# abstractguy/xagents

Hardware: AMD Instinct MI355X
Metric: env-steps/sec/GPU (PPO 16-env) + update ms; 1/2/4/8 MI355X (higher is better)
Workload: dtype f32; 1 GPU; PPO CartPole-v1, 16 envs/GPU, MLP[64,64], n_steps=128, 4 epochs x 4 minibatches, synthetic obs replay (the metric's 16-env configuration); the replay records ignore the actions, so the rollout runs its policy forwards as one batched launch (the `dynamics` object times the sequential step loop of an action-dependent env); n_envs_per_gpu=16, n_steps=128, batch_per_gpu=2048, minibatch_per_gpu=512, ppo_epochs=4, parallelism=dp1, graph=True, train_steps_per_graph_replay=8, update=persistent, allreduce=none

## Files before the change

### xagents_amd/csrc/ppo_tile.hpp

```cpp
#pragma once
#include <type_traits>

#include "ac_tile.hpp"

namespace xa_pt {

using namespace xa_ac;

template <int OBS, int A, int TS>
struct PtLds {
  static constexpr int AH = A + 1, AHP = (AH + 3) & ~3, LDT = TS + 4;
  alignas(16) float sW2[H * LDW];
  alignas(16) float sH1[TS * LDW];
  alignas(16) float sH1T[H * LDT];
  alignas(16) float sdA2[TS * LDW];
  alignas(16) float sZp[4][TS][AHP];
  alignas(16) float sdz[4][TS][AHP];
  alignas(16) float sW1[OBS * H];
  float sb1[H], sb2[H], sW34[H * AH], sb34[AH];
};

template <int OBS, int A>
XA_DEV int canon_of_exchange(int x) {
  const Offs o = offs(OBS, A);
  if (x < H * H) {
    const int pr = x >> 1, t = pr & 255, kk = 2 * (pr >> 8) + (x & 1);
    const int w = t >> 6, lq = (t >> 4) & 3, li = t & 15;
    return o.w2 + (16 * lq + kk) * H + 16 * w + li;
  }
  const int rr = x - H * H;
  return rr < o.w2 ? rr : rr + H * H;
}

template <int OBS, int A>
XA_DEV int exchange_of_rest(int c) {
  const Offs o = offs(OBS, A);
  return H * H + (c < o.w2 ? c : c - H * H);
}

#ifdef XA_NO_REGH1
constexpr bool kRegH1On = false;
#else
constexpr bool kRegH1On = true;
#endif
template <int OBS, int A>
constexpr bool kRegH1 = kRegH1On && OBS == 4 &&
                        1 + (offs(OBS, A).P - offs(OBS, A).b2 + 191) / 192 <= Dims<OBS, A>::RPT;

template <int OBS, int A, int TS>
struct PSlice {
  static constexpr int RPT = Dims<OBS, A>::RPT, NREST = Dims<OBS, A>::NREST;
  int col, row0;
  int ri[RPT];
  int rx[RPT];
  int rdst[RPT];
  XA_DEV static int rest_of(int tid, int q) {
    const Offs o = offs(OBS, A);
    if constexpr (kRegH1<OBS, A>) {
      const int w = tid >> 6, lane = tid & 63, lq = lane >> 4, li = lane & 15, i = 16 * w + li;
      if (q == 0) return o.w1 + lq * H + i;
      if (lq == 0) return q == 1 ? o.b1 + i : -1;
      const int id2 = (lq - 1) * 64 + 16 * w + li, r2 = id2 + 192 * (q - 1);
      return o.b2 + r2 < o.P ? o.b2 + r2 : -1;
    } else {
      const int r = tid + 256 * q;
      return r < NREST ? (r < o.w2 ? r : r + H * H) : -1;
    }
  }
  XA_DEV void init(int tid) {
    const int w = tid >> 6, lane = tid & 63;
    col = 16 * w + (lane & 15);
    row0 = 16 * (lane >> 4);
#pragma unroll
    for (int q = 0; q < RPT; ++q) {
      const int e = rest_of(tid, q);
      ri[q] = e;
      rx[q] = e >= 0 ? exchange_of_rest<OBS, A>(e) : -1;
      rdst[q] = lds_offset_of<PtLds<OBS, A, TS>, OBS, A>(e);
    }
  }
  XA_DEV int w2_canon(int kk) const { return offs(OBS, A).w2 + (row0 + kk) * H + col; }
  XA_DEV void load(const float* base, float (&w)[16], float (&r)[RPT]) const {
#pragma unroll
    for (int kk = 0; kk < 16; ++kk) w[kk] = base[w2_canon(kk)];
#pragma unroll
    for (int q = 0; q < RPT; ++q) r[q] = base[ri[q] >= 0 ? ri[q] : 0];
  }
  XA_DEV void store(float* base, const float (&w)[16], const float (&r)[RPT]) const {
#pragma unroll
    for (int kk = 0; kk < 16; ++kk) base[w2_canon(kk)] = w[kk];
#pragma unroll
    for (int q = 0; q < RPT; ++q)
      if (ri[q] >= 0) base[ri[q]] = r[q];
  }
  XA_DEV void to_lds(PtLds<OBS, A, TS>& L, const float (&w)[16], const float (&r)[RPT]) const {
#pragma unroll
    for (int kk = 0; kk < 16; ++kk) L.sW2[(row0 + kk) * LDW + col] = w[kk];
#pragma unroll
    for (int q = 0; q < RPT; ++q)
      if (rdst[q] >= 0) reinterpret_cast<float*>(&L)[rdst[q]] = r[q];
  }
};

template <int OBS, int A>
struct PtAcc {
  static constexpr int AH = A + 1;
  f32x4 gW2[4];
  float gW34[AH];
  float gW1[OBS];
  float gb1, gb2;
  float gb34[AH];
  float l_pg, l_v, l_ent, l_cnt;
  XA_DEV void zero() {
#pragma unroll
    for (int it = 0; it < 4; ++it) gW2[it] = f32x4{0.0f, 0.0f, 0.0f, 0.0f};
#pragma unroll
    for (int a = 0; a < AH; ++a) gW34[a] = gb34[a] = 0.0f;
#pragma unroll
    for (int k = 0; k < OBS; ++k) gW1[k] = 0.0f;
    gb1 = gb2 = 0.0f;
    l_pg = l_v = l_ent = l_cnt = 0.0f;
  }
};

XA_DEV xa_f2 ftanh2(xa_f2 x) {
  const float c = kTanhClamp;
  const xa_f2 xc = {fminf(fmaxf(x.x, -c), c), fminf(fmaxf(x.y, -c), c)};
  xa_f2 p, q;
  tanh_pq(xc, xc * xc, p, q);
  const xa_f2 r = {__builtin_amdgcn_rcpf(q.x), __builtin_amdgcn_rcpf(q.y)};
  const xa_f2 rn = xa_fma2(xa_fma2(-q, r, xa_f2{1.0f, 1.0f}), r, r);
  return p * rn;
}

XA_DEV float xa_sum16(float v) {
  v = v + XA_DPP_F(v, 0xB1);
  v = v + XA_DPP_F(v, 0x4E);
  v = v + XA_DPP_F(v, 0x141);
  return v + XA_DPP_F(v, 0x140);
}

template <int OBS, int A, int TS>
XA_DEV void load_w2_rows(const PtLds<OBS, A, TS>& L, float (&w2r)[16]) {
  const int tid = threadIdx.x, w = tid >> 6, li = tid & 15, lq = (tid & 63) >> 4;
#pragma unroll
  for (int v4 = 0; v4 < 4; ++v4) {
    const float4 t = *reinterpret_cast<const float4*>(&L.sW2[(16 * w + li) * LDW + 16 * lq + 4 * v4]);
    w2r[4 * v4] = t.x; w2r[4 * v4 + 1] = t.y; w2r[4 * v4 + 2] = t.z; w2r[4 * v4 + 3] = t.w;
  }
}

XA_DEV float2 xa_swap16(float v) {
  const auto a = __builtin_amdgcn_permlane16_swap(__float_as_uint(v), __float_as_uint(v), false, false);
  return make_float2(__uint_as_float(a[0]), __uint_as_float(a[1]));
}
XA_DEV float2 xa_swap32(float v) {
  const auto a = __builtin_amdgcn_permlane32_swap(__float_as_uint(v), __float_as_uint(v), false, false);
  return make_float2(__uint_as_float(a[0]), __uint_as_float(a[1]));
}

struct PtOwnTid {};
template <class PTid>
XA_DEV void pt_pred_lane(PTid ptid, int& pw, int& pli, int& plq) {
  if constexpr (!std::is_same<PTid, PtOwnTid>::value) {
    pw = ptid >> 6;
    pli = ptid & 15;
    plq = (ptid & 63) >> 4;
  }
}

template <int OBS, int A, int TS, class Stamp, class W2Out, class PTid = PtOwnTid>
XA_DEV void pt_tile(PtLds<OBS, A, TS>& L, PtAcc<OBS, A>& acc, const LossCfg& cfg,
                    const float* rec, const float (&w2c)[16], float (&w2r)[16], float w1v,
                    float b1v, Stamp stamp, bool last, W2Out w2_out, PTid ptid = PTid()) {
  static_assert(TS == 16 || TS == 32, "tile sizes: 16 or 32 samples");
  constexpr int NT = TS / 16, AH = A + 1, R = OBS + 4, LDT = PtLds<OBS, A, TS>::LDT;
  const int tid = threadIdx.x, w = tid >> 6, lane = tid & 63;
  const int li = lane & 15, lq = lane >> 4;
  int pw = w, pli = li, plq = lq;
  pt_pred_lane(ptid, pw, pli, plq);
  const int i = 16 * w + li;
  float h1[NT][4];
  {
    float w1[OBS];
    float b1;
    if constexpr (kRegH1<OBS, A>) {
      const float2 s16 = xa_swap16(w1v), s32 = xa_swap32(w1v);
      float vj[4];
      vj[0] = w1v;
      vj[1] = (plq & 1) ? s16.x : s16.y;
      const float2 s48 = xa_swap32(vj[1]);
      vj[2] = (plq & 2) ? s32.x : s32.y;
      vj[3] = (plq & 2) ? s48.x : s48.y;
      const bool o1 = plq & 1, o2 = plq & 2;
#pragma unroll
      for (int k = 0; k < OBS; ++k) {
        const float e0 = ((k & 1) != 0) != o1 ? vj[1] : vj[0];
        const float e1 = ((k & 1) != 0) != o1 ? vj[3] : vj[2];
        w1[k] = ((k & 2) != 0) != o2 ? e1 : e0;
      }
      b1 = xa_swap32(xa_swap16(b1v).x).x;
    } else {
#pragma unroll
      for (int k = 0; k < OBS; ++k) w1[k] = L.sW1[k * H + i];
      b1 = L.sb1[i];
    }
    stamp(47);
#pragma unroll
    for (int mt = 0; mt < NT; ++mt) {
#pragma unroll
      for (int r = 0; r < 4; r += 2) {
        const int s = 16 * mt + 4 * lq + r;
        xa_f2 z = {0.0f, 0.0f};
#pragma unroll
        for (int k = 0; k < OBS; ++k)
          z = xa_fma2(xa_f2{rec[s * R + k], rec[(s + 1) * R + k]}, xa_f2{w1[k], w1[k]}, z);
        const xa_f2 h = ftanh2(z + xa_f2{b1, b1});
        h1[mt][r] = h.x;
        h1[mt][r + 1] = h.y;
      }
      stamp(48);
#pragma unroll
      for (int r = 0; r < 4; ++r) L.sH1[(16 * mt + 4 * lq + r) * LDW + i] = h1[mt][r];
      *reinterpret_cast<float4*>(&L.sH1T[i * LDT + 16 * mt + 4 * lq]) =
          make_float4(h1[mt][0], h1[mt][1], h1[mt][2], h1[mt][3]);
    }
  }
  stamp(49);
  __syncthreads();
  if constexpr (kRegH1<OBS, A>) load_w2_rows(L, w2r);
  stamp(50);
  float h2[NT][4];
  float w34[AH];
#pragma unroll
  for (int a = 0; a < AH; ++a) w34[a] = L.sW34[i * AH + a];
  {
    const float b2 = L.sb2[i];
#pragma unroll
    for (int mt = 0; mt < NT; ++mt) {
      float av[16];
#pragma unroll
      for (int v4 = 0; v4 < 4; ++v4) {
        const float4 t = *reinterpret_cast<const float4*>(&L.sH1[(16 * mt + li) * LDW + 16 * lq + 4 * v4]);
        av[4 * v4] = t.x; av[4 * v4 + 1] = t.y; av[4 * v4 + 2] = t.z; av[4 * v4 + 3] = t.w;
      }
      f32x4 d0 = {0.0f, 0.0f, 0.0f, 0.0f}, d1 = {0.0f, 0.0f, 0.0f, 0.0f};
#pragma unroll
      for (int kk = 0; kk < 16; kk += 2) {
        d0 = mfma4(av[kk], w2c[kk], d0);
        d1 = mfma4(av[kk + 1], w2c[kk + 1], d1);
      }
#pragma unroll
      for (int r = 0; r < 4; r += 2) {
        const xa_f2 h = ftanh2(xa_f2{d0[r], d0[r + 1]} + xa_f2{d1[r], d1[r + 1]} + xa_f2{b2, b2});
        h2[mt][r] = h.x;
        h2[mt][r + 1] = h.y;
      }
    }
  }
  stamp(51);
#pragma unroll
  for (int mt = 0; mt < NT; ++mt)
#pragma unroll
    for (int r = 0; r < 4; ++r)
#pragma unroll
      for (int a = 0; a < AH; ++a) {
        const float p = xa_sum16(h2[mt][r] * w34[a]);
        if (pli == 0) L.sZp[w][16 * mt + 4 * lq + r][a] = p;
      }
  __syncthreads();
  stamp(52);
  constexpr int AHP = PtLds<OBS, A, TS>::AHP;
  const bool tally = pw == 0 && plq == 0;
#pragma unroll
  for (int mt = 0; mt < NT; ++mt) {
    const int s = 16 * mt + li;
    float z[AHP];
#pragma unroll
    for (int a4 = 0; a4 < AHP; a4 += 4) {
      float4 zp[4];
#pragma unroll
      for (int ww = 0; ww < 4; ++ww) zp[ww] = *reinterpret_cast<const float4*>(&L.sZp[ww][s][a4]);
      z[a4] = (zp[0].x + zp[1].x) + (zp[2].x + zp[3].x);
      z[a4 + 1] = (zp[0].y + zp[1].y) + (zp[2].y + zp[3].y);
      z[a4 + 2] = (zp[0].z + zp[1].z) + (zp[2].z + zp[3].z);
      z[a4 + 3] = (zp[0].w + zp[1].w) + (zp[2].w + zp[3].w);
    }
#pragma unroll
    for (int a = 0; a < AH; ++a) z[a] = z[a] + L.sb34[a];
    const float* rs = rec + s * R;
    const float act_f = rs[OBS];
    float dz[AHP];
#pragma unroll
    for (int a = 0; a < AHP; ++a) dz[a] = 0.0f;
    if (act_f >= 0.0f) {
      const int act = (int)act_f;
      float m = z[0];
#pragma unroll
      for (int a = 1; a < A; ++a) m = fmaxf(m, z[a]);
      float e[A], ssum = 0.0f;
#pragma unroll
      for (int a = 0; a < A; ++a) {
        e[a] = fexp(z[a] - m);
        ssum = ssum + e[a];
      }
      const float ls = flog(ssum), rsum = frcp(ssum);
      float lp[A], pr[A], ent = 0.0f, logp = 0.0f;
#pragma unroll
      for (int a = 0; a < A; ++a) {
        lp[a] = (z[a] - m) - ls;
        pr[a] = e[a] * rsum;
        ent = ent - pr[a] * lp[a];
        if (a == act) logp = lp[a];
      }
      const float v = z[A], R_ = rs[OBS + 1], oldv = rs[OBS + 2];
      const float adv = ((R_ - oldv) - cfg.adv_mean) * cfg.adv_rstd;
      const float ratio = fexp(logp - rs[OBS + 3]);
      const float sc = cfg.loss_scale;
      float pg, dlogp, vl, dv;
      ac_loss_terms(true, adv, ratio, logp, v, oldv, R_, cfg.clip_norm, sc, cfg.value_coef, pg,
                    dlogp, vl, dv);
      const float ec = sc * cfg.entropy_coef;
#pragma unroll
      for (int a = 0; a < A; ++a)
        dz[a] = dlogp * ((a == act ? 1.0f : 0.0f) - pr[a]) + ec * pr[a] * (lp[a] + ent);
      dz[A] = dv;
      if (tally) {
        acc.l_pg += pg;
        acc.l_v += vl;
        acc.l_ent += ent;
        acc.l_cnt += 1.0f;
#pragma unroll
        for (int a = 0; a < AH; ++a) acc.gb34[a] += dz[a];
      }
    }
    if (plq == 0) {
#pragma unroll
      for (int a4 = 0; a4 < AHP; a4 += 4)
        *reinterpret_cast<float4*>(&L.sdz[w][s][a4]) = make_float4(dz[a4], dz[a4 + 1], dz[a4 + 2], dz[a4 + 3]);
    }
  }
  __builtin_amdgcn_fence(__ATOMIC_ACQ_REL, "wavefront");
  float da2[NT][4];
#pragma unroll
  for (int mt = 0; mt < NT; ++mt) {
#pragma unroll
    for (int r = 0; r < 4; ++r) {
      const int s = 16 * mt + 4 * lq + r;
      float dz[AHP];
#pragma unroll
      for (int a4 = 0; a4 < AHP; a4 += 4) {
        const float4 t = *reinterpret_cast<const float4*>(&L.sdz[w][s][a4]);
        dz[a4] = t.x; dz[a4 + 1] = t.y; dz[a4 + 2] = t.z; dz[a4 + 3] = t.w;
      }
      float dh = 0.0f;
#pragma unroll
      for (int a = 0; a < AH; ++a) dh = fmaf(dz[a], w34[a], dh);
      const float hv = h2[mt][r];
#pragma unroll
      for (int a = 0; a < AH; ++a) acc.gW34[a] = fmaf(hv, dz[a], acc.gW34[a]);
      const float d = dh * (1.0f - hv * hv);
      acc.gb2 = acc.gb2 + d;
      da2[mt][r] = d;
      L.sdA2[s * LDW + i] = d;
    }
  }
  stamp(53);
#pragma unroll
  for (int it = 0; it < 4; ++it)
#pragma unroll
    for (int mt = 0; mt < NT; ++mt) {
      const float4 t = *reinterpret_cast<const float4*>(&L.sH1T[(16 * it + li) * LDT + 16 * mt + 4 * lq]);
      acc.gW2[it] = mfma4(t.x, da2[mt][0], acc.gW2[it]);
      acc.gW2[it] = mfma4(t.y, da2[mt][1], acc.gW2[it]);
      acc.gW2[it] = mfma4(t.z, da2[mt][2], acc.gW2[it]);
      acc.gW2[it] = mfma4(t.w, da2[mt][3], acc.gW2[it]);
    }
  if (last) w2_out(acc);
  __syncthreads();
  stamp(54);
#pragma unroll
  for (int mt = 0; mt < NT; ++mt) {
    float av[16];
#pragma unroll
    for (int v4 = 0; v4 < 4; ++v4) {
      const float4 t = *reinterpret_cast<const float4*>(&L.sdA2[(16 * mt + li) * LDW + 16 * lq + 4 * v4]);
      av[4 * v4] = t.x; av[4 * v4 + 1] = t.y; av[4 * v4 + 2] = t.z; av[4 * v4 + 3] = t.w;
    }
    f32x4 d0 = {0.0f, 0.0f, 0.0f, 0.0f}, d1 = {0.0f, 0.0f, 0.0f, 0.0f};
#pragma unroll
    for (int kk = 0; kk < 16; kk += 2) {
      d0 = mfma4(av[kk], w2r[kk], d0);
      d1 = mfma4(av[kk + 1], w2r[kk + 1], d1);
    }
#pragma unroll
    for (int r = 0; r < 4; ++r) {
      const int s = 16 * mt + 4 * lq + r;
      const float hv = h1[mt][r];
      const float d = (d0[r] + d1[r]) * (1.0f - hv * hv);
      acc.gb1 = acc.gb1 + d;
#pragma unroll
      for (int k = 0; k < OBS; ++k) acc.gW1[k] = fmaf(rec[s * R + k], d, acc.gW1[k]);
    }
  }
  stamp(55);
}

template <int OBS, int A, class PutPair>
XA_DEV void pt_write_row_w2(const PtAcc<OBS, A>& acc, PutPair put_pair) {
  const int tid = threadIdx.x, w = tid >> 6, lane = tid & 63;
  const int li = lane & 15, lq = lane >> 4;
#pragma unroll
  for (int it = 0; it < 4; ++it) {
    const int t = 64 * w + 16 * it + li;
    put_pair(256 * (2 * lq) + t, acc.gW2[it][0], acc.gW2[it][1]);
    put_pair(256 * (2 * lq + 1) + t, acc.gW2[it][2], acc.gW2[it][3]);
  }
}

template <int OBS, int A, class Put, class PTid = PtOwnTid>
XA_DEV void pt_write_row_rest(PtAcc<OBS, A>& acc, Put put, bool loss_sums = true,
                              PTid ptid = PTid()) {
  constexpr int AH = A + 1;
  const Offs o = offs(OBS, A);
  const int tid = threadIdx.x, w = tid >> 6, lane = tid & 63;
  const int li = lane & 15, lq = lane >> 4;
  const int i = 16 * w + li;
  int pw = w, pli = li, plq = lq;
  pt_pred_lane(ptid, pw, pli, plq);
  auto red = [](float v) {
    const auto a = __builtin_amdgcn_permlane16_swap(__float_as_uint(v), __float_as_uint(v), false, false);
    v = __uint_as_float(a[0]) + __uint_as_float(a[1]);
    const auto c = __builtin_amdgcn_permlane32_swap(__float_as_uint(v), __float_as_uint(v), false, false);
    return __uint_as_float(c[0]) + __uint_as_float(c[1]);
  };
#pragma unroll
  for (int a = 0; a < AH; ++a) acc.gW34[a] = red(acc.gW34[a]);
#pragma unroll
  for (int k = 0; k < OBS; ++k) acc.gW1[k] = red(acc.gW1[k]);
  acc.gb1 = red(acc.gb1);
  acc.gb2 = red(acc.gb2);
  if (pw == 0) {
#pragma unroll
    for (int a = 0; a < AH; ++a) acc.gb34[a] = xa_sum16(acc.gb34[a]);
    if (loss_sums) {
      acc.l_pg = xa_sum16(acc.l_pg);
      acc.l_v = xa_sum16(acc.l_v);
      acc.l_ent = xa_sum16(acc.l_ent);
      acc.l_cnt = xa_sum16(acc.l_cnt);
    }
  }
  if (plq == 0) {
#pragma unroll
    for (int a = 0; a < A; ++a) put(exchange_of_rest<OBS, A>(o.w3 + i * A + a), acc.gW34[a]);
    put(exchange_of_rest<OBS, A>(o.w4 + i), acc.gW34[A]);
    put(exchange_of_rest<OBS, A>(o.b2 + i), acc.gb2);
    put(exchange_of_rest<OBS, A>(o.b1 + i), acc.gb1);
#pragma unroll
    for (int k = 0; k < OBS; ++k) put(exchange_of_rest<OBS, A>(o.w1 + k * H + i), acc.gW1[k]);
    if (pw == 0 && pli == 0) {
#pragma unroll
      for (int a = 0; a < A; ++a) put(exchange_of_rest<OBS, A>(o.b3 + a), acc.gb34[a]);
      put(exchange_of_rest<OBS, A>(o.b4), acc.gb34[A]);
    }
  }
}

}
```

Baseline: 17.39 million env-steps/s.

## Use transposed DPP reduction for head logits and pass dz via row-lane DPP

When the tile holds 16 samples, the per-(row, action) 16-lane DPP sums for the policy/value head are replaced by a transposed butterfly reduction. It reduces 4*AH partial products together, so each lane ends up owning one finished sum and the stores to sZp are spread across lanes. The dz gradients are also kept in registers and broadcast with row_newbcast DPP, instead of being written to and read back from LDS with a wavefront fence. The aim is fewer DPP ops, fewer predicated LDS stores and less LDS round-trip latency in the PPO update. The cost is a more intricate lane-permutation scheme that only applies when TS==16.

```diff
diff --git a/xagents_amd/csrc/ppo_tile.hpp b/xagents_amd/csrc/ppo_tile.hpp
--- a/xagents_amd/csrc/ppo_tile.hpp
+++ b/xagents_amd/csrc/ppo_tile.hpp
@@ -138,6 +138,53 @@
   v = v + XA_DPP_F(v, 0x4E);
   v = v + XA_DPP_F(v, 0x141);
   return v + XA_DPP_F(v, 0x140);
+}
+
+#ifndef XA_PT_TSUM
+#define XA_PT_TSUM 1
+#endif
+#ifndef XA_PT_DZPERM
+#define XA_PT_DZPERM 1
+#endif
+
+XA_DEV int xa_tsum16_index(int li) { return li ^ ((li & 4) ? 3 : 0) ^ ((li & 8) ? 4 : 0); }
+
+template <int K, int N, int NP>
+XA_DEV void xa_tsum16_stage(float (&v)[NP], int e) {
+  constexpr int CTRL = K == 0 ? 0xB1 : K == 1 ? 0x4E : K == 2 ? 0x141 : 0x140;
+  int bit = e & (1 << K);
+  asm volatile("" : "+v"(bit));
+  const bool up = bit != 0;
+#pragma unroll
+  for (int j0 = 0; j0 < NP; j0 += 2 << K) {
+    const int j1 = j0 + (1 << K);
+    if (j0 < N && j1 < N) {
+      const float keep = up ? v[j1] : v[j0], send = up ? v[j0] : v[j1];
+      v[j0] = keep + XA_DPP_F(send, CTRL);
+    } else if (j0 < N) {
+      v[j0] = v[j0] + XA_DPP_F(v[j0], CTRL);
+    }
+  }
+}
+
+template <int N, int NP>
+XA_DEV void xa_tsum16(float (&v)[NP], int e) {
+  static_assert(NP % 16 == 0 && N <= NP && N > NP - 16, "NP = N rounded up to 16 lanes");
+  xa_tsum16_stage<0, N>(v, e);
+  xa_tsum16_stage<1, N>(v, e);
+  xa_tsum16_stage<2, N>(v, e);
+  xa_tsum16_stage<3, N>(v, e);
+}
+
+#define XA_ROW_LANE(v, r) \
+  __int_as_float(__builtin_amdgcn_update_dpp(0, __float_as_int(v), 0x150 + (r), 0xF, 0xF, true))
+XA_DEV float xa_row_lane(float v, int r) {
+  switch (r) {
+    case 0: return XA_ROW_LANE(v, 0);
+    case 1: return XA_ROW_LANE(v, 1);
+    case 2: return XA_ROW_LANE(v, 2);
+    default: return XA_ROW_LANE(v, 3);
+  }
 }
 
 template <int OBS, int A, int TS>
@@ -259,22 +306,38 @@
     }
   }
   stamp(51);
-#pragma unroll
-  for (int mt = 0; mt < NT; ++mt)
-#pragma unroll
-    for (int r = 0; r < 4; ++r)
-#pragma unroll
-      for (int a = 0; a < AH; ++a) {
-        const float p = xa_sum16(h2[mt][r] * w34[a]);
-        if (pli == 0) L.sZp[w][16 * mt + 4 * lq + r][a] = p;
-      }
+  constexpr bool kTsum = XA_PT_TSUM && TS == 16, kDzPerm = XA_PT_DZPERM && TS == 16;
+  if constexpr (kTsum) {
+    constexpr int NP = (4 * AH + 15) & ~15;
+    static_assert(NP / 4 <= PtLds<OBS, A, TS>::AHP, "the padding columns take the rest");
+    float p[NP];
+#pragma unroll
+    for (int a = 0; a < AH; ++a)
+#pragma unroll
+      for (int r = 0; r < 4; ++r) p[4 * a + r] = h2[0][r] * w34[a];
+    xa_tsum16<4 * AH>(p, xa_tsum16_index(pli));
+    const int e = xa_tsum16_index(li);
+#pragma unroll
+    for (int c = 0; c < NP / 16; ++c) L.sZp[w][4 * lq + (e & 3)][4 * c + (e >> 2)] = p[16 * c];
+  } else {
+#pragma unroll
+    for (int mt = 0; mt < NT; ++mt)
+#pragma unroll
+      for (int r = 0; r < 4; ++r)
+#pragma unroll
+        for (int a = 0; a < AH; ++a) {
+          const float p = xa_sum16(h2[mt][r] * w34[a]);
+          if (pli == 0) L.sZp[w][16 * mt + 4 * lq + r][a] = p;
+        }
+  }
   __syncthreads();
   stamp(52);
   constexpr int AHP = PtLds<OBS, A, TS>::AHP;
   const bool tally = pw == 0 && plq == 0;
+  [[maybe_unused]] float dzl[AH];
 #pragma unroll
   for (int mt = 0; mt < NT; ++mt) {
-    const int s = 16 * mt + li;
+    const int s = kDzPerm ? ((li + 4 * lq) & 15) : 16 * mt + li;
     float z[AHP];
 #pragma unroll
     for (int a4 = 0; a4 < AHP; a4 += 4) {
@@ -334,13 +397,16 @@
         for (int a = 0; a < AH; ++a) acc.gb34[a] += dz[a];
       }
     }
-    if (plq == 0) {
+    if constexpr (kDzPerm) {
+#pragma unroll
+      for (int a = 0; a < AH; ++a) dzl[a] = dz[a];
+    } else if (plq == 0) {
 #pragma unroll
       for (int a4 = 0; a4 < AHP; a4 += 4)
         *reinterpret_cast<float4*>(&L.sdz[w][s][a4]) = make_float4(dz[a4], dz[a4 + 1], dz[a4 + 2], dz[a4 + 3]);
     }
   }
-  __builtin_amdgcn_fence(__ATOMIC_ACQ_REL, "wavefront");
+  if constexpr (!kDzPerm) __builtin_amdgcn_fence(__ATOMIC_ACQ_REL, "wavefront");
   float da2[NT][4];
 #pragma unroll
   for (int mt = 0; mt < NT; ++mt) {
@@ -348,10 +414,15 @@
     for (int r = 0; r < 4; ++r) {
       const int s = 16 * mt + 4 * lq + r;
       float dz[AHP];
-#pragma unroll
-      for (int a4 = 0; a4 < AHP; a4 += 4) {
-        const float4 t = *reinterpret_cast<const float4*>(&L.sdz[w][s][a4]);
-        dz[a4] = t.x; dz[a4 + 1] = t.y; dz[a4 + 2] = t.z; dz[a4 + 3] = t.w;
+      if constexpr (kDzPerm) {
+#pragma unroll
+        for (int a = 0; a < AH; ++a) dz[a] = xa_row_lane(dzl[a], r);
+      } else {
+#pragma unroll
+        for (int a4 = 0; a4 < AHP; a4 += 4) {
+          const float4 t = *reinterpret_cast<const float4*>(&L.sdz[w][s][a4]);
+          dz[a4] = t.x; dz[a4 + 1] = t.y; dz[a4 + 2] = t.z; dz[a4 + 3] = t.w;
+        }
       }
       float dh = 0.0f;
 #pragma unroll
```

Result: faster. 18.55 million env-steps/s, median of 6 (+6.6%).
